# netease-youdao/EmotiVoice

Measured on AMD Instinct MI355X. Metric: mel_frames_per_sec, higher is better.
Workload: dtype f16+mxfp4 (fp32-class activations travelling as plane sets; per product one fp16 MFMA on the hi parts + two block-scaled MFMAs for the cross terms: fp4 x fp4 in every generator stage, the decoder's conv-FFN and QKV / output projections, fp4 weights x E5M2 activations in the fused 32-channel k = 3 pa

## Files before the change

emotivoice_amd/csrc/ev_gemm.hip:

```cpp
#include <hip/hip_fp16.h>
#include <stdlib.h>

#include "ev_kernels.h"
#include "ev_mxq.h"

#pragma clang fp contract(off)

namespace ev {

typedef _Float16 half8 __attribute__((ext_vector_type(8)));
typedef float f32x4 __attribute__((ext_vector_type(4)));
typedef float f32x2 __attribute__((ext_vector_type(2)));
typedef _Float16 half2v __attribute__((ext_vector_type(2)));

static constexpr int MAX_SPAN = 64;

__device__ __forceinline__ float max_raw(float a, float b) {
    float r;
    asm("v_max_f32 %0, %1, %2" : "=v"(r) : "v"(a), "v"(b));
    return r;
}
__device__ __forceinline__ float min_raw(float a, float b) {
    float r;
    asm("v_min_f32 %0, %1, %2" : "=v"(r) : "v"(a), "v"(b));
// ... 193 lines not shown
#define EV_TRACE_EPI_PARAMS
#define EV_TRACE_EPI_ARGS
#define EV_TRACE_EPI_DUMMY
#define EV_STAMP()
#endif

enum { EPI_RES16 = 1, EPI_RES32 = 2, EPI_ACC32 = 4, EPI_GENERIC = 8, EPI_RARE_ACT = 16, EPI_O16 = 32, EPI_O32 = 64, EPI_ADD16 = 128, EPI_LEAN = 256,
       EPI_MXP = 512, EPI_RESPL = 1024, EPI_ACCPL = 2048, EPI_PART = 4096 };

__device__ __forceinline__ float quad_xor1(float v) { return __builtin_bit_cast(float, __builtin_amdgcn_mov_dpp(__builtin_bit_cast(int, v), 0xB1, 0xF, 0xF, true)); }
__device__ __forceinline__ float quad_xor2(float v) { return __builtin_bit_cast(float, __builtin_amdgcn_mov_dpp(__builtin_bit_cast(int, v), 0x4E, 0xF, 0xF, true)); }
__device__ __forceinline__ void mx_quant8(const f32x2 (&a)[4], uint4& ho, unsigned& ch, unsigned& cl, unsigned& bh, unsigned& bl) {
    half2v hh[4];
    f32x2 hf[4], lf[4];
    float mh = 0.f, ml = 0.f;
#pragma unroll
    for (int j = 0; j < 4; ++j) {
        hh[j] = __builtin_convertvector(a[j], half2v);
        hf[j] = __builtin_convertvector(hh[j], f32x2);
        lf[j] = a[j] - hf[j];
        mh = max3_abs_raw(hf[j][0], hf[j][1], mh);
        ml = max3_abs_raw(lf[j][0], lf[j][1], ml);
    }
    mh = max_raw(mh, quad_xor1(mh)); mh = max_raw(mh, quad_xor2(mh));
    ml = max_raw(ml, quad_xor1(ml)); ml = max_raw(ml, quad_xor2(ml));
    bh = mx_scale_byte(mh); bl = mx_scale_byte(ml);
    const float sh = __uint_as_float(bh << 23), sl = __uint_as_float(bl << 23);
    ch = 0; cl = 0;
    ch = __builtin_amdgcn_cvt_scalef32_pk_fp4_f32(ch, hf[0][0], hf[0][1], sh, 0); cl = __builtin_amdgcn_cvt_scalef32_pk_fp4_f32(cl, lf[0][0], lf[0][1], sl, 0);
    ch = __builtin_amdgcn_cvt_scalef32_pk_fp4_f32(ch, hf[1][0], hf[1][1], sh, 1); cl = __builtin_amdgcn_cvt_scalef32_pk_fp4_f32(cl, lf[1][0], lf[1][1], sl, 1);
    ch = __builtin_amdgcn_cvt_scalef32_pk_fp4_f32(ch, hf[2][0], hf[2][1], sh, 2); cl = __builtin_amdgcn_cvt_scalef32_pk_fp4_f32(cl, lf[2][0], lf[2][1], sl, 2);
    ch = __builtin_amdgcn_cvt_scalef32_pk_fp4_f32(ch, hf[3][0], hf[3][1], sh, 3); cl = __builtin_amdgcn_cvt_scalef32_pk_fp4_f32(cl, lf[3][0], lf[3][1], sl, 3);
    ho.x = *reinterpret_cast<unsigned*>(&hh[0]); ho.y = *reinterpret_cast<unsigned*>(&hh[1]);
    ho.z = *reinterpret_cast<unsigned*>(&hh[2]); ho.w = *reinterpret_cast<unsigned*>(&hh[3]);
}
__device__ __forceinline__ long mx_scale_offset(const ConvGemmParams& p, long lin, long row_, int co) {
    const long row = p.mxo_logC ? (lin >> p.mxo_logC) : row_;
    const unsigned c = p.mxo_logC ? ((unsigned)lin & ((1u << p.mxo_logC) - 1u)) : (unsigned)co;
    return (long)(c >> 7) * p.mxo_qs_stride + row * 4 + ((c >> 5) & 3);
}
template <typename T>
__device__ __forceinline__ T* uptr(T* q) {
    unsigned long long b = reinterpret_cast<unsigned long long>(q);
    asm("" : "+s"(b));
    typedef __attribute__((address_space(1))) T* gptr;
    return (T*)(gptr)b;
}
__device__ __forceinline__ unsigned vlane(unsigned x) { asm volatile("" : "+v"(x)); return x; }
template <bool PART = false>
__device__ __forceinline__ void mx_emit_planes(const ConvGemmParams& p, const f32x2 (&a)[4], long ulin, unsigned llin_, long uso, unsigned lso_, int lane) {
    uint4 ho;
    unsigned ch, cl, bh, bl;
    mx_quant8(a, ho, ch, cl, bh, bl);
    const unsigned lh = vlane(llin_ * 2u), lq = vlane(llin_ >> 1), lso = vlane(lso_);
    char* const ph = uptr(reinterpret_cast<char*>(p.mxo_h) + ulin * 2);
    char* const pq0 = uptr(reinterpret_cast<char*>(p.mxo_q4[0]) + (ulin >> 1));
    char* const pq1 = uptr(reinterpret_cast<char*>(p.mxo_q4[1]) + (ulin >> 1));
#ifdef EV_MX_ABL
    const int abl = p.reserved0 >> 4;
    if (abl & 4) { if (p.M < 0) *reinterpret_cast<uint4*>(ph + lh) = uint4{ho.x ^ ch, ho.y ^ cl, ho.z ^ bh, ho.w ^ bl}; return; }
    if (abl & 8) { if (p.M < 0) ho.x ^= ch ^ cl ^ bh ^ bl; *reinterpret_cast<uint4*>(ph + lh) = ho; return; }
    if (abl & 16) {
        if (p.M < 0) ho.x ^= bh ^ bl;
        *reinterpret_cast<uint4*>(ph + lh) = ho;
        *reinterpret_cast<unsigned*>(pq0 + lq) = ch;
        *reinterpret_cast<unsigned*>(pq1 + lq) = cl;
        return;
    }
#endif
    *reinterpret_cast<uint4*>(ph + lh) = ho;
    if constexpr (!PART) *reinterpret_cast<unsigned*>(pq0 + lq) = ch;
    *reinterpret_cast<unsigned*>(pq1 + lq) = cl;
    if ((lane & 3) == 0) {
        if constexpr (!PART) uptr(reinterpret_cast<uint8_t*>(p.mxo_qs[0]) + uso)[lso] = (uint8_t)bh;
        uptr(reinterpret_cast<uint8_t*>(p.mxo_qs[1]) + uso)[lso] = (uint8_t)bl;
    }
}
__device__ __forceinline__ long uniform64(long v) {
    const unsigned lo = (unsigned)__builtin_amdgcn_readfirstlane((int)(unsigned)v), hi = (unsigned)__builtin_amdgcn_readfirstlane((int)(unsigned)((unsigned long)v >> 32));
    return (long)(((unsigned long)hi << 32) | lo);
}
__device__ uint8_t g_row_always_valid[4] = {1, 1, 1, 1};

template <int MT, int NT, int EPI, int RP = 32>
__device__ __forceinline__ void gemm_epilogue_fast(const ConvGemmParams& p, f32x4 (&acc)[NT][MT], char* wave_lds, int t0, int co0 EV_TRACE_EPI_PARAMS) {
    constexpr int TC = NT * 16;
    constexpr bool SWZ = RP == 16;
    constexpr int PITCH = SWZ ? TC * 4 : epi_pitch<TC>();
#ifdef EV_MXT
    unsigned long long mxt_e[12];
    int mxt_i = 0;
#define EV_MXT_STAMP() { __builtin_amdgcn_sched_barrier(0); mxt_e[mxt_i++] = __builtin_readcyclecounter(); __builtin_amdgcn_sched_barrier(0); }
#else
#define EV_MXT_STAMP()
#endif
    EV_MXT_STAMP()
    constexpr int LPR = TC / 8, RPI = 64 / LPR, IT = RP / RPI, NP = MT * 16 / RP, NG = MT / 2;
    static_assert((RP == 32 || (RP == 16 && TC == 64)) && IT >= 1, "rows per pass");
    int lane_ = threadIdx.x & 63;
    if constexpr (SWZ) asm volatile("" : "+v"(lane_));
    const int lane = lane_;
    const int fr = lane & 15, fq = lane >> 4;
    const int rr = lane / LPR, g = lane % LPR;
    const int co = co0 + g * 8;
    const int trow = t0 + rr;
    const int t0u = __builtin_amdgcn_readfirstlane(t0), co0u = __builtin_amdgcn_readfirstlane(co0);
    const unsigned l_o0 = (unsigned)(rr * p.ldo + g * 8), l_res0 = (unsigned)(rr * p.ldres + g * 8), l_acc0 = (unsigned)(rr * p.ldacc + g * 8),
                   l_add0 = (unsigned)(rr * p.ldadd + g * 8);
    const unsigned b_o32 = l_o0 * 4u, b_o16 = l_o0 * 2u, b_res16 = l_res0 * 2u, b_res32 = l_res0 * 4u, b_resq = l_res0 >> 1, b_acc = l_acc0 * 4u, b_add = l_add0 * 2u;
    const unsigned b_acc16 = l_acc0 * 2u, b_accq = l_acc0 >> 1;

    const uint8_t* vptr = p.row_valid ? p.row_valid : g_row_always_valid;
    const int vshift = p.row_valid ? p.valid_shift : 31;
    uint8_t vld[NG];
#pragma unroll
    for (int pass = 0; pass < NG; ++pass) vld[pass] = vptr[(t0 + pass * 32 + (lane & 31)) >> vshift];
    uint4 r16[2][IT], a16[2][IT][2];
    float4 r32[2][IT][2], a32[2][IT][2];
    uint4 rph[2][IT];
    unsigned rpc[2][IT], rps[2][IT];
    long rp_su = 0;
    unsigned rp_sl0 = 0;
    if constexpr (EPI & EPI_RESPL) {
        const long so = (long)(co >> 7) * p.res_xs_stride + ((co >> 5) & 3) + (long)rr * 4;
        rp_su = uniform64(so) + (long)t0u * 4;
        rp_sl0 = (unsigned)(so - uniform64(so));
    }
    uint4 aph[2][IT];
    unsigned apc[2][IT], aps[2][IT];
    long ap_su = 0;
    unsigned ap_sl0 = 0;
    if constexpr (EPI & EPI_ACCPL) {
        const long so = (long)(co >> 7) * p.acc_xs_stride + ((co >> 5) & 3) + (long)rr * 4;
        ap_su = uniform64(so) + (long)t0u * 4;
        ap_sl0 = (unsigned)(so - uniform64(so));
    }
    constexpr bool LEAN = (EPI & EPI_LEAN) != 0;
#define EV_EPI_RD(IT_, H) (SWZ ? ((IT_) * RPI + rr) * PITCH + (((2 * g + (H)) ^ (((IT_) * RPI + rr) & 15)) << 4) : ((IT_) * RPI + rr) * PITCH + g * 32 + (H) * 16)
#define EV_EPI_SET(PASS) (LEAN ? 0 : ((PASS) & 1))
#define EV_EPI_PREFETCH(PASS)                                                                                              \
    _Pragma("unroll") for (int it = 0; it < IT; ++it) {                                                                    \
        const long tu_ = t0u + (PASS) * RP + it * RPI;                                                                     \
        if constexpr (EPI & EPI_RES16)                                                                                     \
            r16[EV_EPI_SET(PASS)][it] = *reinterpret_cast<const uint4*>(uptr(reinterpret_cast<const char*>(p.res) + (tu_ * p.ldres + co0u) * 2) + vlane(b_res16)); \
        if constexpr (EPI & EPI_RES32) {                                                                                   \
            const char* rp_ = uptr(reinterpret_cast<const char*>(p.res) + (tu_ * p.ldres + co0u) * 4) + vlane(b_res32);    \
            r32[EV_EPI_SET(PASS)][it][0] = *reinterpret_cast<const float4*>(rp_);                                          \
            r32[EV_EPI_SET(PASS)][it][1] = *reinterpret_cast<const float4*>(rp_ + 16);                                     \
        }                                                                                                                  \
        if constexpr (EPI & EPI_RESPL) {                                                                                   \
            const long ulin_ = tu_ * p.ldres + co0u;                                                                       \
            rph[EV_EPI_SET(PASS)][it] = *reinterpret_cast<const uint4*>(uptr(reinterpret_cast<const char*>(p.res) + ulin_ * 2) + vlane(b_res16));  \
            rpc[EV_EPI_SET(PASS)][it] = *reinterpret_cast<const unsigned*>(uptr(reinterpret_cast<const char*>(p.res_x4) + (ulin_ >> 1)) + vlane(b_resq)); \
            rps[EV_EPI_SET(PASS)][it] = uptr(reinterpret_cast<const uint8_t*>(p.res_xs) + (rp_su + ((PASS) * RP + it * RPI) * 4))[vlane(rp_sl0)]; \
        }                                                                                                                  \
        if constexpr (EPI & EPI_ACCPL) {                                                                                   \
            const long ulin_ = tu_ * p.ldacc + co0u;                                                                       \
            aph[EV_EPI_SET(PASS)][it] = *reinterpret_cast<const uint4*>(uptr(reinterpret_cast<const char*>(p.acc_h) + ulin_ * 2) + vlane(b_acc16));  \
            apc[EV_EPI_SET(PASS)][it] = *reinterpret_cast<const unsigned*>(uptr(reinterpret_cast<const char*>(p.acc_x4) + (ulin_ >> 1)) + vlane(b_accq)); \
            aps[EV_EPI_SET(PASS)][it] = uptr(reinterpret_cast<const uint8_t*>(p.acc_xs) + (ap_su + ((PASS) * RP + it * RPI) * 4))[vlane(ap_sl0)]; \
        }                                                                                                                  \
        if constexpr (EPI & EPI_ACC32) {                                                                                   \
            const char* ap_ = uptr(reinterpret_cast<const char*>(p.acc32) + (tu_ * p.ldacc + co0u) * 4) + vlane(b_acc);    \
            a32[EV_EPI_SET(PASS)][it][0] = *reinterpret_cast<const float4*>(ap_);                                          \
            a32[EV_EPI_SET(PASS)][it][1] = *reinterpret_cast<const float4*>(ap_ + 16);                                     \
        }                                                                                                                  \
        if constexpr (EPI & EPI_ADD16) {                                                                                   \
            a16[EV_EPI_SET(PASS)][it][0] = *reinterpret_cast<const uint4*>(uptr(reinterpret_cast<const char*>(p.add16_a) + (tu_ * p.ldadd + co0u) * 2) + vlane(b_add)); \
            a16[EV_EPI_SET(PASS)][it][1] = *reinterpret_cast<const uint4*>(uptr(reinterpret_cast<const char*>(p.add16_b) + (tu_ * p.ldadd + co0u) * 2) + vlane(b_add)); \
        }                                                                                                                  \
    }
    if constexpr (!LEAN) { EV_EPI_PREFETCH(0) }
    unsigned vmask[NG];
#pragma unroll
    for (int pass = 0; pass < NG; ++pass) vmask[pass] = (unsigned)__builtin_amdgcn_ballot_w64(vld[pass] != 0);

    f32x2 bias2[4];
#pragma unroll
    for (int j = 0; j < 4; ++j) bias2[j] = f32x2{0.f, 0.f};
    if (p.bias) {
        const float4 b0 = *reinterpret_cast<const float4*>(p.bias + co), b1 = *reinterpret_cast<const float4*>(p.bias + co + 4);
        bias2[0] = f32x2{b0.x, b0.y}; bias2[1] = f32x2{b0.z, b0.w}; bias2[2] = f32x2{b1.x, b1.y}; bias2[3] = f32x2{b1.z, b1.w};
    }
    const int act = p.act;
    const f32x2 act_slope2 = f32x2{p.act_slope, p.act_slope};
    const f32x2 out_scale2 = f32x2{p.out_scale, p.out_scale};
    const bool has_post = p.post_lrelu != 0;
    const f32x2 post_slope2 = f32x2{p.post_slope, p.post_slope};
    const f32x2 mxo_slope2 = f32x2{p.mxo_slope, p.mxo_slope};
    const f32x2 res_inv2 = f32x2{p.res_inv_slope, p.res_inv_slope};
    const bool mxo_act = __float_as_uint(p.mxo_slope) != 0x3f800000u, scaled = __float_as_uint(p.out_scale) != 0x3f800000u;
    __half* const o16 = reinterpret_cast<__half*>(p.out16);
    float* const o32a = p.out32_before_post ? p.out32 : nullptr;
    float* const o32b = p.out32_before_post ? nullptr : p.out32;
    const long rowoff_u = (long)t0u * p.ldo + co0u;
    unsigned lrbit[32 / RPI];
#pragma unroll
    for (int it = 0; it < 32 / RPI; ++it) lrbit[it] = 1u << (it * RPI + rr);
    long mx_su = 0;
    unsigned mx_sl = 0;
    int mx_sstep = 0;
    if constexpr (EPI & EPI_MXP) {
        static_assert(TC == 64, "plane-set epilogue: 64-channel wave tiles");
        const long so = mx_scale_offset(p, rowoff_u + l_o0, (long)trow, co);
        mx_su = uniform64(so);
        mx_sl = (unsigned)(so - mx_su);
        mx_sstep = 4 * (p.mxo_logC ? (p.ldo >> p.mxo_logC) : 1);
    }
    EV_STAMP()
    EV_MXT_STAMP()

#pragma unroll
    for (int pass = 0; pass < NP; ++pass) {
#ifdef EV_MXT
        if constexpr (SWZ) {
            if (p.reserved0 & 4) {
                const bool late = (threadIdx.x >> 8) != 0;
                if (pass == 0) { if (late) __builtin_amdgcn_s_setprio(1); }
                if (pass == NP / 2) { if (late) __builtin_amdgcn_s_setprio(0); else __builtin_amdgcn_s_setprio(1); }
            }
        }
#endif
        __builtin_amdgcn_wave_barrier();
        if constexpr (LEAN) { EV_EPI_PREFETCH(pass) }
        if constexpr (SWZ) {
#pragma unroll
            for (int a = 0; a < NT; ++a)
                *reinterpret_cast<f32x4*>(wave_lds + fr * PITCH + (((a * 4 + fq) ^ fr) << 4)) = acc[a][pass];
        } else {
#pragma unroll
            for (int bb = 0; bb < 2; ++bb)
#pragma unroll
                for (int a = 0; a < NT; ++a)
                    *reinterpret_cast<f32x4*>(wave_lds + (bb * 16 + fr) * PITCH + (a * 16 + 4 * fq) * 4) = acc[a][pass * 2 + bb];
        }
        __builtin_amdgcn_wave_barrier();
        if constexpr (!LEAN) { if (pass + 1 < NP) { EV_EPI_PREFETCH(pass + 1) } }
        EV_STAMP()
        f32x4 lv[IT][2];
        if constexpr (!LEAN) {
#pragma unroll
            for (int it = 0; it < IT; ++it) {
                lv[it][0] = *reinterpret_cast<const f32x4*>(wave_lds + EV_EPI_RD(it, 0));
                lv[it][1] = *reinterpret_cast<const f32x4*>(wave_lds + EV_EPI_RD(it, 1));
            }
        }
#pragma unroll
        for (int it = 0; it < IT; ++it) {
            if constexpr (LEAN) {
                lv[it][0] = *reinterpret_cast<const f32x4*>(wave_lds + EV_EPI_RD(it, 0));
                lv[it][1] = *reinterpret_cast<const f32x4*>(wave_lds + EV_EPI_RD(it, 1));
            }
            const long off_u = rowoff_u + (long)(pass * RP + it * RPI) * p.ldo;
            const f32x4 v0 = lv[it][0], v1 = lv[it][1];
            f32x2 v[4] = {f32x2{v0[0], v0[1]}, f32x2{v0[2], v0[3]}, f32x2{v1[0], v1[1]}, f32x2{v1[2], v1[3]}};
#pragma unroll
            for (int j = 0; j < 4; ++j) v[j] += bias2[j];
            if constexpr (EPI & EPI_RARE_ACT) {
                if (act == ACT_GELU && (EPI & (EPI_O16 | EPI_MXP)) && !(EPI & EPI_O32)) {
#pragma unroll
                    for (int j = 0; j < 4; ++j) { v[j][0] = gelu_fast(v[j][0]); v[j][1] = gelu_fast(v[j][1]); }
                } else {
#pragma unroll
                    for (int j = 0; j < 4; ++j) { v[j][0] = apply_act(v[j][0], act, 0.f); v[j][1] = apply_act(v[j][1], act, 0.f); }
                }
            } else if (act == ACT_LRELU) {
#pragma unroll
                for (int j = 0; j < 4; ++j) v[j] = lrelu2(v[j], act_slope2);
            }
            if constexpr (EPI & EPI_RES16) {
                const half2v* h = reinterpret_cast<const half2v*>(&r16[EV_EPI_SET(pass)][it]);
#pragma unroll
                for (int j = 0; j < 4; ++j) v[j] += __builtin_convertvector(h[j], f32x2);
            }
            if constexpr (EPI & EPI_RES32) {
                const float4 r0 = r32[EV_EPI_SET(pass)][it][0], r1 = r32[EV_EPI_SET(pass)][it][1];
                v[0] += f32x2{r0.x, r0.y}; v[1] += f32x2{r0.z, r0.w}; v[2] += f32x2{r1.x, r1.y}; v[3] += f32x2{r1.z, r1.w};
            }
            if constexpr (EPI & EPI_RESPL) {
                const half2v* h = reinterpret_cast<const half2v*>(&rph[EV_EPI_SET(pass)][it]);
                const unsigned cw = rpc[EV_EPI_SET(pass)][it];
                const float sc = __uint_as_float(rps[EV_EPI_SET(pass)][it] << 23);
                f32x2 a[4];
                a[0] = __builtin_convertvector(h[0], f32x2) + __builtin_amdgcn_cvt_scalef32_pk_f32_fp4(cw, sc, 0);
                a[1] = __builtin_convertvector(h[1], f32x2) + __builtin_amdgcn_cvt_scalef32_pk_f32_fp4(cw, sc, 1);
                a[2] = __builtin_convertvector(h[2], f32x2) + __builtin_amdgcn_cvt_scalef32_pk_f32_fp4(cw, sc, 2);
                a[3] = __builtin_convertvector(h[3], f32x2) + __builtin_amdgcn_cvt_scalef32_pk_f32_fp4(cw, sc, 3);
#pragma unroll
                for (int j = 0; j < 4; ++j) {
                    const f32x2 t = a[j] * res_inv2;
                    v[j] += f32x2{min_raw(a[j][0], t[0]), min_raw(a[j][1], t[1])};
                }
            }
            if (scaled) {
                asm volatile("" ::: "memory");
#pragma unroll
                for (int j = 0; j < 4; ++j) v[j] *= out_scale2;
            }
            if constexpr (EPI & EPI_ACC32) {
                const float4 r0 = a32[EV_EPI_SET(pass)][it][0], r1 = a32[EV_EPI_SET(pass)][it][1];
                v[0] += f32x2{r0.x, r0.y}; v[1] += f32x2{r0.z, r0.w}; v[2] += f32x2{r1.x, r1.y}; v[3] += f32x2{r1.z, r1.w};
            }
            if constexpr (EPI & EPI_ACCPL) {
                const half2v* h = reinterpret_cast<const half2v*>(&aph[EV_EPI_SET(pass)][it]);
                const unsigned cw = apc[EV_EPI_SET(pass)][it];
// ... 1858 lines not shown
```

emotivoice_amd/csrc/ev_gemm_mx64.h:

```cpp
#pragma once

template <int TAPS>
struct Mx64Sched {
    static constexpr int KG = (TAPS + 1) / 2, KH = (KG + 1) / 2, KP = KG * 2, NS = 2 * KG + 2 * KH;
    static constexpr int chunk_of(int s) { return s < KG ? 0 : (s < 2 * KG ? 1 : (s < 2 * KG + KH ? 2 : 3)); }
    static constexpr int first_of(int c) { return c == 0 ? 0 : (c == 1 ? KG : (c == 2 ? 2 * KG : 2 * KG + KH)); }
    static constexpr bool starts_chunk(int s) { return s == first_of(chunk_of(s)); }
    static constexpr int x_issued(int t) { return (starts_chunk(t) && chunk_of(t) < 3) ? 3 : 0; }
    static constexpr int w_issued(int t) { return t + 3 < NS ? 1 : 0; }
    static constexpr int issued_before(int t) {
        int n = 6;
        for (int j = 0; j < t; ++j) n += x_issued(j) + w_issued(j);
        return n;
    }
    static constexpr int idx_w(int m) { return m < 3 ? 3 + m : issued_before(m - 3) + x_issued(m - 3); }
    static constexpr int idx_xlast(int c) { return c == 0 ? 2 : issued_before(first_of(c - 1)) + 2; }
    static constexpr int wait_imm(int s) {
        if (s + 1 >= NS) return -1;
        int need = idx_w(s + 1);
        if (starts_chunk(s + 1)) { const int x = idx_xlast(chunk_of(s + 1)); need = x > need ? x : need; }
        return issued_before(s) - 1 - need;
    }
};
static_assert(Mx64Sched<11>::NS == 18 && Mx64Sched<7>::NS == 12 && Mx64Sched<11>::wait_imm(0) == 1 && Mx64Sched<11>::wait_imm(1) == 4 && Mx64Sched<11>::wait_imm(2) == 1, "schedule");

template <int N> __device__ __forceinline__ void mx64_wait() {
    if constexpr (N >= 0) asm volatile("s_waitcnt vmcnt(%0)" ::"n"(N) : "memory");
}

template <int TAPS, int EPI>
__global__ __launch_bounds__(512, 4) void conv_gemm_mx64_kernel(const ConvGemmParams p) {
    using SC = Mx64Sched<TAPS>;
    constexpr int BM = PH_BM, XBUF = PH_XBUF, WBUF = PH_WBUF, MT = 2, NT = 4, KG = SC::KG, KP = SC::KP, NS = SC::NS;
    static_assert(PH_SLABR >= BM + MAX_SPAN + 64 && KP * 128 <= 2048 && (TAPS == 7 || TAPS == 11), "slab rows / weight-scale run / tap counts");
    extern __shared__ __attribute__((aligned(16))) char smem[];
    char* const Xs = smem;
    char* const Ws = smem + 2 * XBUF;
    const int tid = threadIdx.x, lane = tid & 63;
    const int wave = __builtin_amdgcn_readfirstlane(tid >> 6);
    const int wc = wave >> 2;
    const unsigned lds0 = (unsigned)(size_t)(__attribute__((address_space(3))) char*)smem;

    int bid = blockIdx.x;
    {
        const int nblk = gridDim.x, q = nblk >> 3, r = nblk & 7, xcd = bid & 7, local = bid >> 3;
        bid = (xcd < r ? xcd * (q + 1) : r * (q + 1) + (xcd - r) * q) + local;
    }
    const int m0 = bid * BM;
    const int dil = p.dil;
    const int row0 = m0 - p.center * dil;
    const int row0a = row0 & ~3, soff = row0 - row0a;
    const int last_row = BM + (TAPS - 1) * dil - 1;

    const int prow = lane >> 2;
    const unsigned pp16 = (unsigned)(((lane & 3) ^ ((lane >> 3) & 3)) << 4);
    const int wco = (wave & 3) * 16 + prow;
    const unsigned w16_lane = (unsigned)wco * (unsigned)(TAPS * 128) + pp16;
    const unsigned wq = (unsigned)((lane & 3) ^ ((lane >> 3) & 3));
    const unsigned w4_lane = (unsigned)(((wco >> 5) * KP + (int)(wq >> 1)) * 1024 + (wco & 31) * 32 + (int)(wq & 1) * 16);
    unsigned x16_lane[3], x4_lane[2];
#pragma unroll
    for (int i = 0; i < 3; ++i) x16_lane[i] = (unsigned)min((wave + 8 * i) * 16 + prow, last_row) * 128u + pp16;
#pragma unroll
    for (int i = 0; i < 2; ++i) x4_lane[i] = (unsigned)min((wave + 8 * i) * 32 + (lane >> 1), last_row) * 32u + (unsigned)(lane & 1) * 16u;
    const int xs_run = ((BM + (TAPS - 1) * dil + soff) * 4 + 15) & ~15;
    unsigned sc_lane;
    if (wave == 4) sc_lane = min(lane * 16, xs_run - 16);
    else if (wave == 5) sc_lane = min(1024 + lane * 16, xs_run - 16);
    else if (wave == 6) sc_lane = min(lane * 16, KP * 128 - 16);
    else sc_lane = min(1024 + lane * 16, KP * 128 - 16);

    const char* const wmx = reinterpret_cast<const char*>(p.W_mx);
    constexpr int WQB = KP * 32 * 32 * 2, WSB = KP * 32 * 2 * 2;
    const char* const xb16 = uniform_ptr(reinterpret_cast<const char*>(p.A) + (long)row0 * 128L);
    const char* const xb4[2] = {uniform_ptr(reinterpret_cast<const char*>(p.mx_x4[0]) + (long)row0 * 32L), uniform_ptr(reinterpret_cast<const char*>(p.mx_x4[1]) + (long)row0 * 32L)};
    const char* const xsb[2] = {uniform_ptr(reinterpret_cast<const char*>(p.mx_xs[0]) + (long)row0a * 4L), uniform_ptr(reinterpret_cast<const char*>(p.mx_xs[1]) + (long)row0a * 4L)};
    const char* const wb16 = uniform_ptr(reinterpret_cast<const char*>(p.W));
    const unsigned xdst = __builtin_amdgcn_readfirstlane(lds0 + wave * 1024), wdst = xdst + 2 * XBUF;

    auto issue_x = [&](auto cc) {
        constexpr int C_ = decltype(cc)::value;
        constexpr unsigned dst = (unsigned)((C_ & 1) * XBUF);
        if constexpr (C_ < 2) {
#pragma unroll
            for (int i = 0; i < 3; ++i) glds16(xb16 + C_ * 64, x16_lane[i], xdst + dst + i * 8192);
        } else {
            constexpr int P_ = C_ - 2;
            glds16(xb4[P_], x4_lane[0], xdst + dst);
            glds16(xb4[P_], x4_lane[1], xdst + dst + 8192);
            const bool sc = wave >= 4;
            const char* const sbase = wave < 6 ? xsb[P_] : wmx + 2 * WQB + P_ * WSB;
            glds16(sc ? sbase : xb4[P_], sc ? sc_lane : x4_lane[1], xdst + dst + 2 * 8192);
        }
    };
    auto issue_w = [&](auto ss) {
        constexpr int S_ = decltype(ss)::value;
        constexpr int C_ = SC::chunk_of(S_), U_ = S_ - SC::first_of(C_);
        const int sel = wave >> 2;
        if constexpr (C_ < 2) {
            const int t = min(2 * U_ + sel, TAPS - 1);
            glds16(wb16 + C_ * 64 + (unsigned)t * 128u, w16_lane, wdst + (S_ & 3) * WBUF);
        } else {
            const int g = min(2 * U_ + sel, KG - 1);
            glds16(wmx + (C_ - 2) * WQB + (unsigned)(2 * g) * 1024u, w4_lane, wdst + (S_ & 3) * WBUF);
        }
    };

    f32x4 acc[NT][MT];
#pragma unroll
    for (int a = 0; a < NT; ++a)
#pragma unroll
        for (int b = 0; b < MT; ++b) acc[a][b] = f32x4{0.f, 0.f, 0.f, 0.f};
    const int fr = lane & 15, fq = lane >> 4;

    bool tile_live = true;
    if (p.row_valid) {
        const uint8_t* vp = p.row_valid;
        const int r4 = m0 + lane * 4, vs = p.valid_shift;
        const unsigned any = vp[r4 >> vs] | vp[(r4 + 1) >> vs] | vp[(r4 + 2) >> vs] | vp[(r4 + 3) >> vs];
        tile_live = __builtin_amdgcn_ballot_w64(any != 0) != 0ull;
    }
    if (tile_live) {
        issue_x(std::integral_constant<int, 0>{});
        issue_w(std::integral_constant<int, 0>{});
        issue_w(std::integral_constant<int, 1>{});
        issue_w(std::integral_constant<int, 2>{});
        asm volatile("s_waitcnt vmcnt(0)" ::: "memory");
        __builtin_amdgcn_s_barrier();
        if (wc == 1) __builtin_amdgcn_s_barrier();

        const int xrow = wave * 32 + fr;
        const int x4row = xrow + (fq >> 1) * dil;
        const int xs_base = MX_XS_OFF + soff * 4 + (fq & 1);
        int ws_lane[NT];
#pragma unroll
        for (int a = 0; a < NT; ++a) {
            const int co = a * 16 + fr;
            ws_lane[a] = MX_WS_OFF + (((co >> 5) * KP + (fq >> 1)) * 32 + (co & 31)) * 2 + (fq & 1);
        }

#define EV_MX64_STEP(S)                                                                                                              \
    if constexpr ((S) < NS) {                                                                                                        \
        constexpr int C_ = SC::chunk_of(S), U_ = (S) - SC::first_of(C_);                                                             \
        const char* const Xb = Xs + (C_ & 1) * XBUF;                                                                                 \
        const char* const Wb = Ws + ((S) & 3) * WBUF;                                                                                \
        uint4 xf[2][MT], wf[2][NT];                                                                                                  \
        int xsc[2][MT], wsc[2][NT];                                                                                                  \
        constexpr int NSEL = (C_ < 2) ? ((2 * U_ + 1 < TAPS) ? 2 : 1) : ((2 * U_ + 1 < KG) ? 2 : 1);                                 \
        int dil_ = dil;                                                                                                              \
        asm volatile("" : "+s"(dil_));                                                                                               \
        _Pragma("unroll") for (int sel = 0; sel < NSEL; ++sel) {                                                                     \
            _Pragma("unroll") for (int a = 0; a < NT; ++a) wf[sel][a] = *reinterpret_cast<const uint4*>(Wb + swz(sel * 64 + a * 16 + fr, fq)); \
            if constexpr (C_ < 2) {                                                                                                  \
                const int r_ = xrow + (2 * U_ + sel) * dil_;                                                                         \
                _Pragma("unroll") for (int b = 0; b < MT; ++b) {                                                                     \
                    const int rb_ = r_ + b * 16;                                                                                     \
                    xf[sel][b] = *reinterpret_cast<const uint4*>(Xb + rb_ * 64 + ((fq ^ ((rb_ >> 1) & 3)) << 4));                    \
                }                                                                                                                    \
            } else {                                                                                                                 \
                const int g_ = 2 * U_ + sel;                                                                                         \
                const int r_ = x4row + 2 * g_ * dil_;                                                                                \
                _Pragma("unroll") for (int b = 0; b < MT; ++b) {                                                                     \
                    xf[sel][b] = *reinterpret_cast<const uint4*>(Xb + (r_ + b * 16) * 32 + ((fq & 1) << 4));                         \
                    xsc[sel][b] = *reinterpret_cast<const uint8_t*>(Xb + xs_base + (r_ + b * 16) * 4);                               \
                }                                                                                                                    \
                _Pragma("unroll") for (int a = 0; a < NT; ++a) wsc[sel][a] = *reinterpret_cast<const uint8_t*>(Xb + ws_lane[a] + g_ * 128); \
            }                                                                                                                        \
        }                                                                                                                            \
        mx64_wait<SC::wait_imm(S)>();                                                                                                \
        __builtin_amdgcn_sched_barrier(0);                                                                                           \
        __builtin_amdgcn_s_barrier();                                                                                                \
        __builtin_amdgcn_sched_barrier(0);                                                                                           \
        __builtin_amdgcn_s_setprio(1);                                                                                               \
        _Pragma("unroll") for (int sel = 0; sel < NSEL; ++sel)                                                                       \
            _Pragma("unroll") for (int a = 0; a < NT; ++a)                                                                           \
                _Pragma("unroll") for (int b = 0; b < MT; ++b) {                                                                     \
                    if constexpr (C_ < 2) mfma_inplace(acc[a][b], *reinterpret_cast<half8*>(&wf[sel][a]), *reinterpret_cast<half8*>(&xf[sel][b])); \
                    else mfma_mx_inplace(acc[a][b], wf[sel][a], xf[sel][b], wsc[sel][a], xsc[sel][b]);                               \
                    const int idx = (sel * NT + a) * MT + b;                                                                         \
                    if constexpr (SC::x_issued(S) != 0) { if (idx == 2) issue_x(std::integral_constant<int, (C_ < 3 ? C_ + 1 : 3)>{}); } \
                    if constexpr (SC::w_issued(S) != 0) { if (idx == 5) issue_w(std::integral_constant<int, ((S) + 3 < NS ? (S) + 3 : 0)>{}); } \
                }                                                                                                                    \
        __builtin_amdgcn_s_setprio(0);                                                                                               \
        __builtin_amdgcn_sched_barrier(0);                                                                                           \
        __builtin_amdgcn_s_barrier();                                                                                                \
        __builtin_amdgcn_sched_barrier(0);                                                                                           \
    }
        EV_MX64_STEP(0) EV_MX64_STEP(1) EV_MX64_STEP(2) EV_MX64_STEP(3) EV_MX64_STEP(4) EV_MX64_STEP(5)
        EV_MX64_STEP(6) EV_MX64_STEP(7) EV_MX64_STEP(8) EV_MX64_STEP(9) EV_MX64_STEP(10) EV_MX64_STEP(11)
        EV_MX64_STEP(12) EV_MX64_STEP(13) EV_MX64_STEP(14) EV_MX64_STEP(15) EV_MX64_STEP(16) EV_MX64_STEP(17)
#undef EV_MX64_STEP
        asm volatile("s_waitcnt vmcnt(0)" ::: "memory");
        if (wc == 0) __builtin_amdgcn_s_barrier();
        __builtin_amdgcn_s_barrier();
        mfma_asm_fence(acc);
    }
    if constexpr (EPI == EPI_GENERIC) gemm_epilogue_lds<MT, NT>(p, acc, smem + wave * epi_wave_bytes<64>(), m0 + wave * 32, 0);
    else {
        EV_TRACE_EPI_DUMMY
        gemm_epilogue_fast<MT, NT, EPI, 16>(p, acc, smem + wave * 4096, m0 + wave * 32, 0 EV_TRACE_EPI_ARGS);
    }
}

template <int TAPS, int EPI>
static void launch_mx64_epi(const ConvGemmParams& p, hipStream_t s) {
    hipLaunchKernelGGL((conv_gemm_mx64_kernel<TAPS, EPI>), dim3(p.M / PH_BM), dim3(512), PH_LDS, s, p);
}
template <int TAPS>
static void launch_mx64_taps(const ConvGemmParams& p, int e, hipStream_t s) {
    switch (e) {
#define EV_MX64_CASE(E) case (E): launch_mx64_epi<TAPS, (E)>(p, s); break;
        EV_MX_VARIANTS(EV_MX64_CASE)
#undef EV_MX64_CASE
        default: break;
    }
}
template <int TAPS>
static hipError_t mx64_attr_taps() {
    hipError_t e = hipSuccess, r;
#define EV_MX64_ATTR(E) r = hipFuncSetAttribute((const void*)conv_gemm_mx64_kernel<TAPS, (E)>, hipFuncAttributeMaxDynamicSharedMemorySize, (int)PH_LDS); if (r != hipSuccess) e = r;
    EV_MX_VARIANTS(EV_MX64_ATTR)
#undef EV_MX64_ATTR
    return e;
}
static hipError_t mx64_set_attributes() {
    hipError_t e = hipSuccess, r;
    r = mx64_attr_taps<7>(); if (r != hipSuccess) e = r;
    r = mx64_attr_taps<11>(); if (r != hipSuccess) e = r;
    return e;
}
static bool mx64_eligible(const ConvGemmParams& p) {
    return p.W_mx && p.N == 64 && p.K == 64 && p.lda == 64 && (p.taps == 11 || p.taps == 7) && p.M % PH_BM == 0 && (p.taps - 1) * p.dil <= MAX_SPAN &&
           p.center * 2 == p.taps - 1 && p.mx_x4[0] && p.mx_x4[1] && p.mx_xs[0] && p.mx_xs[1] && !p.pro_lrelu && !(p.reserved0 & 8) && mx_epi_variant(p) >= 0;
}
static void launch_mx64(const ConvGemmParams& p, hipStream_t s) {
    if (p.taps == 7) launch_mx64_taps<7>(p, mx_epi_variant(p), s); else launch_mx64_taps<11>(p, mx_epi_variant(p), s);
}
```

Before: 726,900.

## Add 384-row tile variant of mx64 conv GEMM with reworked load schedule

```diff
diff --git a/emotivoice_amd/csrc/ev_gemm.hip b/emotivoice_amd/csrc/ev_gemm.hip
--- a/emotivoice_amd/csrc/ev_gemm.hip
+++ b/emotivoice_amd/csrc/ev_gemm.hip
@@ -299,7 +299,7 @@
 }
 __device__ uint8_t g_row_always_valid[4] = {1, 1, 1, 1};
 
-template <int MT, int NT, int EPI, int RP = 32>
+template <int MT, int NT, int EPI, int RP = 32, bool MLIM = false>
 __device__ __forceinline__ void gemm_epilogue_fast(const ConvGemmParams& p, f32x4 (&acc)[NT][MT], char* wave_lds, int t0, int co0 EV_TRACE_EPI_PARAMS) {
     constexpr int TC = NT * 16;
     constexpr bool SWZ = RP == 16;
@@ -312,8 +312,8 @@
 #define EV_MXT_STAMP()
 #endif
     EV_MXT_STAMP()
-    constexpr int LPR = TC / 8, RPI = 64 / LPR, IT = RP / RPI, NP = MT * 16 / RP, NG = MT / 2;
-    static_assert((RP == 32 || (RP == 16 && TC == 64)) && IT >= 1, "rows per pass");
+    constexpr int LPR = TC / 8, RPI = 64 / LPR, IT = RP / RPI, NP = MT * 16 / RP, NG = (MT + 1) / 2;
+    static_assert((RP == 32 || (RP == 16 && TC == 64)) && IT >= 1 && (MT % 2 == 0 || RP == 16) && (!MLIM || RP == 16), "rows per pass");
     int lane_ = threadIdx.x & 63;
     if constexpr (SWZ) asm volatile("" : "+v"(lane_));
     const int lane = lane_;
@@ -331,7 +331,7 @@
     const int vshift = p.row_valid ? p.valid_shift : 31;
     uint8_t vld[NG];
 #pragma unroll
-    for (int pass = 0; pass < NG; ++pass) vld[pass] = vptr[(t0 + pass * 32 + (lane & 31)) >> vshift];
+    for (int pass = 0; pass < NG; ++pass) vld[pass] = vptr[(MLIM ? min(t0 + pass * 32 + (lane & 31), p.M - 1) : t0 + pass * 32 + (lane & 31)) >> vshift];
     uint4 r16[2][IT], a16[2][IT][2];
     float4 r32[2][IT][2], a32[2][IT][2];
     uint4 rph[2][IT];
@@ -357,7 +357,8 @@
 #define EV_EPI_SET(PASS) (LEAN ? 0 : ((PASS) & 1))
 #define EV_EPI_PREFETCH(PASS)                                                                                              \
     _Pragma("unroll") for (int it = 0; it < IT; ++it) {                                                                    \
-        const long tu_ = t0u + (PASS) * RP + it * RPI;                                                                     \
+        const int du_ = MLIM ? min(t0u + (PASS) * RP + it * RPI, p.M - RPI) - t0u : (PASS) * RP + it * RPI;                \
+        const long tu_ = t0u + du_;                                                                                        \
         if constexpr (EPI & EPI_RES16)                                                                                     \
             r16[EV_EPI_SET(PASS)][it] = *reinterpret_cast<const uint4*>(uptr(reinterpret_cast<const char*>(p.res) + (tu_ * p.ldres + co0u) * 2) + vlane(b_res16)); \
         if constexpr (EPI & EPI_RES32) {                                                                                   \
@@ -369,13 +370,13 @@
             const long ulin_ = tu_ * p.ldres + co0u;                                                                       \
             rph[EV_EPI_SET(PASS)][it] = *reinterpret_cast<const uint4*>(uptr(reinterpret_cast<const char*>(p.res) + ulin_ * 2) + vlane(b_res16));  \
             rpc[EV_EPI_SET(PASS)][it] = *reinterpret_cast<const unsigned*>(uptr(reinterpret_cast<const char*>(p.res_x4) + (ulin_ >> 1)) + vlane(b_resq)); \
-            rps[EV_EPI_SET(PASS)][it] = uptr(reinterpret_cast<const uint8_t*>(p.res_xs) + (rp_su + ((PASS) * RP + it * RPI) * 4))[vlane(rp_sl0)]; \
+            rps[EV_EPI_SET(PASS)][it] = uptr(reinterpret_cast<const uint8_t*>(p.res_xs) + (rp_su + du_ * 4))[vlane(rp_sl0)]; \
         }                                                                                                                  \
         if constexpr (EPI & EPI_ACCPL) {                                                                                   \
             const long ulin_ = tu_ * p.ldacc + co0u;                                                                       \
             aph[EV_EPI_SET(PASS)][it] = *reinterpret_cast<const uint4*>(uptr(reinterpret_cast<const char*>(p.acc_h) + ulin_ * 2) + vlane(b_acc16));  \
             apc[EV_EPI_SET(PASS)][it] = *reinterpret_cast<const unsigned*>(uptr(reinterpret_cast<const char*>(p.acc_x4) + (ulin_ >> 1)) + vlane(b_accq)); \
-            aps[EV_EPI_SET(PASS)][it] = uptr(reinterpret_cast<const uint8_t*>(p.acc_xs) + (ap_su + ((PASS) * RP + it * RPI) * 4))[vlane(ap_sl0)]; \
+            aps[EV_EPI_SET(PASS)][it] = uptr(reinterpret_cast<const uint8_t*>(p.acc_xs) + (ap_su + du_ * 4))[vlane(ap_sl0)]; \
         }                                                                                                                  \
         if constexpr (EPI & EPI_ACC32) {                                                                                   \
             const char* ap_ = uptr(reinterpret_cast<const char*>(p.acc32) + (tu_ * p.ldacc + co0u) * 4) + vlane(b_acc);    \
@@ -438,6 +439,7 @@
             }
         }
 #endif
+        if constexpr (MLIM) { if (t0u + pass * RP >= p.M) break; }
         __builtin_amdgcn_wave_barrier();
         if constexpr (LEAN) { EV_EPI_PREFETCH(pass) }
         if constexpr (SWZ) {
diff --git a/emotivoice_amd/csrc/ev_gemm_mx64.h b/emotivoice_amd/csrc/ev_gemm_mx64.h
--- a/emotivoice_amd/csrc/ev_gemm_mx64.h
+++ b/emotivoice_amd/csrc/ev_gemm_mx64.h
@@ -1,20 +1,23 @@
 #pragma once
 
-template <int TAPS>
+template <int TAPS, int MT_ = 2>
 struct Mx64Sched {
     static constexpr int KG = (TAPS + 1) / 2, KH = (KG + 1) / 2, KP = KG * 2, NS = 2 * KG + 2 * KH;
+    static constexpr int XP16 = MT_ == 3 ? 4 : 3, XP4 = 3, WD = MT_ == 3 ? 2 : 3;
+    static constexpr bool W_FIRST = MT_ == 3;
+    static constexpr int pieces(int c) { return c < 2 ? XP16 : XP4; }
     static constexpr int chunk_of(int s) { return s < KG ? 0 : (s < 2 * KG ? 1 : (s < 2 * KG + KH ? 2 : 3)); }
     static constexpr int first_of(int c) { return c == 0 ? 0 : (c == 1 ? KG : (c == 2 ? 2 * KG : 2 * KG + KH)); }
     static constexpr bool starts_chunk(int s) { return s == first_of(chunk_of(s)); }
-    static constexpr int x_issued(int t) { return (starts_chunk(t) && chunk_of(t) < 3) ? 3 : 0; }
-    static constexpr int w_issued(int t) { return t + 3 < NS ? 1 : 0; }
+    static constexpr int x_issued(int t) { return (starts_chunk(t) && chunk_of(t) < 3) ? pieces(chunk_of(t) + 1) : 0; }
+    static constexpr int w_issued(int t) { return t + WD < NS ? 1 : 0; }
     static constexpr int issued_before(int t) {
-        int n = 6;
+        int n = pieces(0) + WD;
         for (int j = 0; j < t; ++j) n += x_issued(j) + w_issued(j);
         return n;
     }
-    static constexpr int idx_w(int m) { return m < 3 ? 3 + m : issued_before(m - 3) + x_issued(m - 3); }
-    static constexpr int idx_xlast(int c) { return c == 0 ? 2 : issued_before(first_of(c - 1)) + 2; }
+    static constexpr int idx_w(int m) { return m < WD ? pieces(0) + m : issued_before(m - WD) + (W_FIRST ? 0 : x_issued(m - WD)); }
+    static constexpr int idx_xlast(int c) { return c == 0 ? pieces(0) - 1 : issued_before(first_of(c - 1)) + (W_FIRST ? w_issued(first_of(c - 1)) : 0) + pieces(c) - 1; }
     static constexpr int wait_imm(int s) {
         if (s + 1 >= NS) return -1;
         int need = idx_w(s + 1);
@@ -23,16 +26,22 @@
     }
 };
 static_assert(Mx64Sched<11>::NS == 18 && Mx64Sched<7>::NS == 12 && Mx64Sched<11>::wait_imm(0) == 1 && Mx64Sched<11>::wait_imm(1) == 4 && Mx64Sched<11>::wait_imm(2) == 1, "schedule");
+static_assert(Mx64Sched<11, 3>::wait_imm(0) == 0 && Mx64Sched<11, 3>::wait_imm(1) == 4 && Mx64Sched<11, 3>::wait_imm(2) == 0 && Mx64Sched<11, 3>::wait_imm(5) == 0 &&
+              Mx64Sched<7, 3>::wait_imm(1) == 4 && Mx64Sched<7, 3>::wait_imm(3) == 0, "schedule, 384 rows");
+
+static constexpr int MX64_XBUF384 = (384 + MAX_SPAN) * 64;
 
 template <int N> __device__ __forceinline__ void mx64_wait() {
     if constexpr (N >= 0) asm volatile("s_waitcnt vmcnt(%0)" ::"n"(N) : "memory");
 }
 
-template <int TAPS, int EPI>
+template <int TAPS, int EPI, int MT = 2>
 __global__ __launch_bounds__(512, 4) void conv_gemm_mx64_kernel(const ConvGemmParams p) {
-    using SC = Mx64Sched<TAPS>;
-    constexpr int BM = PH_BM, XBUF = PH_XBUF, WBUF = PH_WBUF, MT = 2, NT = 4, KG = SC::KG, KP = SC::KP, NS = SC::NS;
-    static_assert(PH_SLABR >= BM + MAX_SPAN + 64 && KP * 128 <= 2048 && (TAPS == 7 || TAPS == 11), "slab rows / weight-scale run / tap counts");
+    using SC = Mx64Sched<TAPS, MT>;
+    constexpr bool R384 = MT == 3;
+    constexpr int BM = MT * 128, XBUF = R384 ? MX64_XBUF384 : PH_XBUF, WBUF = PH_WBUF, NT = 4, KG = SC::KG, KP = SC::KP, NS = SC::NS, NSLOT = SC::WD + 1;
+    static_assert((MT == 2 || MT == 3) && XBUF >= (BM + MAX_SPAN) * 64 && (BM + MAX_SPAN) * 32 <= 16384 && (BM + MAX_SPAN + 3) * 4 <= 2048 && MX_XS_OFF + 4096 <= XBUF &&
+                  2 * XBUF + NSLOT * WBUF <= (int)PH_LDS && KP * 128 <= 2048 && (TAPS == 7 || TAPS == 11), "slab rows / scale runs / LDS / tap counts");
     extern __shared__ __attribute__((aligned(16))) char smem[];
     char* const Xs = smem;
     char* const Ws = smem + 2 * XBUF;
@@ -50,7 +59,8 @@
     const int dil = p.dil;
     const int row0 = m0 - p.center * dil;
     const int row0a = row0 & ~3, soff = row0 - row0a;
-    const int last_row = BM + (TAPS - 1) * dil - 1;
+    const int tile_rows = R384 ? min(BM, p.M - m0) : BM;
+    const int last_row = tile_rows + (TAPS - 1) * dil - 1;
 
     const int prow = lane >> 2;
     const unsigned pp16 = (unsigned)(((lane & 3) ^ ((lane >> 3) & 3)) << 4);
@@ -58,12 +68,14 @@
     const unsigned w16_lane = (unsigned)wco * (unsigned)(TAPS * 128) + pp16;
     const unsigned wq = (unsigned)((lane & 3) ^ ((lane >> 3) & 3));
     const unsigned w4_lane = (unsigned)(((wco >> 5) * KP + (int)(wq >> 1)) * 1024 + (wco & 31) * 32 + (int)(wq & 1) * 16);
-    unsigned x16_lane[3], x4_lane[2];
-#pragma unroll
-    for (int i = 0; i < 3; ++i) x16_lane[i] = (unsigned)min((wave + 8 * i) * 16 + prow, last_row) * 128u + pp16;
+    constexpr int XP16 = SC::XP16;
+    const int x16_p3 = wave >= 4 ? 2 : 3;
+    unsigned x16_lane[XP16], x4_lane[2];
+#pragma unroll
+    for (int i = 0; i < XP16; ++i) x16_lane[i] = (unsigned)min((wave + 8 * (i == 3 ? x16_p3 : i)) * 16 + prow, last_row) * 128u + pp16;
 #pragma unroll
     for (int i = 0; i < 2; ++i) x4_lane[i] = (unsigned)min((wave + 8 * i) * 32 + (lane >> 1), last_row) * 32u + (unsigned)(lane & 1) * 16u;
-    const int xs_run = ((BM + (TAPS - 1) * dil + soff) * 4 + 15) & ~15;
+    const int xs_run = ((tile_rows + (TAPS - 1) * dil + soff) * 4 + 15) & ~15;
     unsigned sc_lane;
     if (wave == 4) sc_lane = min(lane * 16, xs_run - 16);
     else if (wave == 5) sc_lane = min(1024 + lane * 16, xs_run - 16);
@@ -83,7 +95,7 @@
         constexpr unsigned dst = (unsigned)((C_ & 1) * XBUF);
         if constexpr (C_ < 2) {
 #pragma unroll
-            for (int i = 0; i < 3; ++i) glds16(xb16 + C_ * 64, x16_lane[i], xdst + dst + i * 8192);
+            for (int i = 0; i < XP16; ++i) glds16(xb16 + C_ * 64, x16_lane[i], xdst + dst + (i == 3 ? x16_p3 : i) * 8192);
         } else {
             constexpr int P_ = C_ - 2;
             glds16(xb4[P_], x4_lane[0], xdst + dst);
@@ -99,10 +111,10 @@
         const int sel = wave >> 2;
         if constexpr (C_ < 2) {
             const int t = min(2 * U_ + sel, TAPS - 1);
-            glds16(wb16 + C_ * 64 + (unsigned)t * 128u, w16_lane, wdst + (S_ & 3) * WBUF);
+            glds16(wb16 + C_ * 64 + (unsigned)t * 128u, w16_lane, wdst + (S_ % NSLOT) * WBUF);
         } else {
             const int g = min(2 * U_ + sel, KG - 1);
-            glds16(wmx + (C_ - 2) * WQB + (unsigned)(2 * g) * 1024u, w4_lane, wdst + (S_ & 3) * WBUF);
+            glds16(wmx + (C_ - 2) * WQB + (unsigned)(2 * g) * 1024u, w4_lane, wdst + (S_ % NSLOT) * WBUF);
         }
     };
 
@@ -111,25 +123,40 @@
     for (int a = 0; a < NT; ++a)
 #pragma unroll
         for (int b = 0; b < MT; ++b) acc[a][b] = f32x4{0.f, 0.f, 0.f, 0.f};
+    if constexpr (R384) {
+#pragma unroll
+        for (int a = 0; a < NT; ++a)
+#pragma unroll
+            for (int b = 0; b < MT; ++b) asm volatile("" : "+v"(acc[a][b]));
+    }
     const int fr = lane & 15, fq = lane >> 4;
 
     bool tile_live = true;
     if (p.row_valid) {
         const uint8_t* vp = p.row_valid;
-        const int r4 = m0 + lane * 4, vs = p.valid_shift;
-        const unsigned any = vp[r4 >> vs] | vp[(r4 + 1) >> vs] | vp[(r4 + 2) >> vs] | vp[(r4 + 3) >> vs];
+        const int vs = p.valid_shift;
+        unsigned any;
+        if constexpr (R384) {
+            const int r6 = m0 + lane * 6, rl = p.M - 1;
+            any = 0;
+#pragma unroll
+            for (int i = 0; i < 6; ++i) any |= vp[min(r6 + i, rl) >> vs];
+        } else {
+            const int r4 = m0 + lane * 4;
+            any = vp[r4 >> vs] | vp[(r4 + 1) >> vs] | vp[(r4 + 2) >> vs] | vp[(r4 + 3) >> vs];
+        }
         tile_live = __builtin_amdgcn_ballot_w64(any != 0) != 0ull;
     }
     if (tile_live) {
         issue_x(std::integral_constant<int, 0>{});
         issue_w(std::integral_constant<int, 0>{});
         issue_w(std::integral_constant<int, 1>{});
-        issue_w(std::integral_constant<int, 2>{});
+        if constexpr (SC::WD > 2) issue_w(std::integral_constant<int, 2>{});
         asm volatile("s_waitcnt vmcnt(0)" ::: "memory");
         __builtin_amdgcn_s_barrier();
         if (wc == 1) __builtin_amdgcn_s_barrier();
 
-        const int xrow = wave * 32 + fr;
+        const int xrow = wave * (MT * 16) + fr;
         const int x4row = xrow + (fq >> 1) * dil;
         const int xs_base = MX_XS_OFF + soff * 4 + (fq & 1);
         int ws_lane[NT];
@@ -143,7 +170,7 @@
     if constexpr ((S) < NS) {                                                                                                        \
         constexpr int C_ = SC::chunk_of(S), U_ = (S) - SC::first_of(C_);                                                             \
         const char* const Xb = Xs + (C_ & 1) * XBUF;                                                                                 \
-        const char* const Wb = Ws + ((S) & 3) * WBUF;                                                                                \
+        const char* const Wb = Ws + ((S) % NSLOT) * WBUF;                                                                            \
         uint4 xf[2][MT], wf[2][NT];                                                                                                  \
         int xsc[2][MT], wsc[2][NT];                                                                                                  \
         constexpr int NSEL = (C_ < 2) ? ((2 * U_ + 1 < TAPS) ? 2 : 1) : ((2 * U_ + 1 < KG) ? 2 : 1);                                 \
@@ -186,19 +213,87 @@
         __builtin_amdgcn_s_barrier();                                                                                                \
         __builtin_amdgcn_sched_barrier(0);                                                                                           \
     }
+#define EV_MX64_LDW(SEL, A_)                                                                                                         \
+        { wf[A_] = *reinterpret_cast<const uint4*>(Wb + swz((SEL) * 64 + (A_) * 16 + fr, fq));                                       \
+          if constexpr (C_ >= 2) wsc[A_] = *reinterpret_cast<const uint8_t*>(Xb + ws_lane[A_] + (2 * U_ + (SEL)) * 128); }
+#define EV_MX64_LDX(DST, DSC, SEL, B_)                                                                                               \
+        { if constexpr (C_ < 2) {                                                                                                    \
+              const int rb_ = xrow + (2 * U_ + (SEL)) * dil_ + (B_) * 16;                                                            \
+              DST = *reinterpret_cast<const uint4*>(Xb + rb_ * 64 + ((fq ^ ((rb_ >> 1) & 3)) << 4));                                 \
+          } else {                                                                                                                   \
+              const int rb_ = x4row + 2 * (2 * U_ + (SEL)) * dil_ + (B_) * 16;                                                       \
+              DST = *reinterpret_cast<const uint4*>(Xb + rb_ * 32 + ((fq & 1) << 4));                                                \
+              DSC = *reinterpret_cast<const uint8_t*>(Xb + xs_base + rb_ * 4);                                                       \
+          } }
+#define EV_MX64_MMA(A_, XF, XS)                                                                                                      \
+        { if constexpr (C_ < 2) mfma_inplace(acc[A_][b], *reinterpret_cast<half8*>(&wf[A_]), *reinterpret_cast<half8*>(&XF));         \
+          else mfma_mx_inplace(acc[A_][b], wf[A_], XF, wsc[A_], XS); }
+#define EV_MX64_STEP3(S)                                                                                                             \
+    if constexpr ((S) < NS) {                                                                                                        \
+        constexpr int C_ = SC::chunk_of(S), U_ = (S) - SC::first_of(C_);                                                             \
+        const char* const Xb = Xs + (C_ & 1) * XBUF;                                                                                 \
+        const char* const Wb = Ws + ((S) % NSLOT) * WBUF;                                                                            \
+        uint4 xf[MT], xg[MT], wf[NT];                                                                                                \
+        int xsc[MT], xgc[MT], wsc[NT];                                                                                               \
+        constexpr int NSEL = (C_ < 2) ? ((2 * U_ + 1 < TAPS) ? 2 : 1) : ((2 * U_ + 1 < KG) ? 2 : 1);                                 \
+        int dil_ = dil;                                                                                                              \
+        asm volatile("" : "+s"(dil_));                                                                                               \
+        _Pragma("unroll") for (int a = 0; a < NT; ++a) EV_MX64_LDW(0, a)                                                             \
+        _Pragma("unroll") for (int b = 0; b < MT; ++b) EV_MX64_LDX(xf[b], xsc[b], 0, b)                                              \
+        mx64_wait<SC::wait_imm(S)>();                                                                                                \
+        __builtin_amdgcn_sched_barrier(0);                                                                                           \
+        __builtin_amdgcn_s_barrier();                                                                                                \
+        __builtin_amdgcn_sched_barrier(0);                                                                                           \
+        __builtin_amdgcn_s_setprio(1);                                                                                               \
+        _Pragma("unroll") for (int a = 0; a < NT; ++a) {                                                                             \
+            _Pragma("unroll") for (int b = 0; b < MT; ++b) {                                                                         \
+                EV_MX64_MMA(a, xf[b], xsc[b])                                                                                        \
+                const int idx = a * MT + b;                                                                                          \
+                if constexpr (SC::w_issued(S) != 0) { if (idx == 1) issue_w(std::integral_constant<int, ((S) + SC::WD < NS ? (S) + SC::WD : 0)>{}); } \
+                if constexpr (SC::x_issued(S) != 0) { if (idx == 4) issue_x(std::integral_constant<int, (C_ < 3 ? C_ + 1 : 3)>{}); } \
+            }                                                                                                                        \
+            if constexpr (NSEL == 2) {                                                                                               \
+                __builtin_amdgcn_sched_barrier(0);                                                                                   \
+                EV_MX64_LDW(1, a)                                                                                                    \
+                if (a == NT - 2) EV_MX64_LDX(xg[0], xgc[0], 1, 0)                                                                    \
+                if (a == NT - 1) { _Pragma("unroll") for (int b = 1; b < MT; ++b) EV_MX64_LDX(xg[b], xgc[b], 1, b) }                 \
+                __builtin_amdgcn_sched_barrier(0);                                                                                   \
+            }                                                                                                                        \
+        }                                                                                                                            \
+        if constexpr (NSEL == 2) {                                                                                                   \
+            _Pragma("unroll") for (int b = 0; b < MT; ++b)                                                                           \
+                _Pragma("unroll") for (int a = 0; a < NT; ++a) EV_MX64_MMA(a, xg[b], xgc[b])                                         \
+        }                                                                                                                            \
+        __builtin_amdgcn_s_setprio(0);                                                                                               \
+        __builtin_amdgcn_sched_barrier(0);                                                                                           \
+        __builtin_amdgcn_s_barrier();                                                                                                \
+        __builtin_amdgcn_sched_barrier(0);                                                                                           \
+    }
+        if constexpr (!R384) {
         EV_MX64_STEP(0) EV_MX64_STEP(1) EV_MX64_STEP(2) EV_MX64_STEP(3) EV_MX64_STEP(4) EV_MX64_STEP(5)
         EV_MX64_STEP(6) EV_MX64_STEP(7) EV_MX64_STEP(8) EV_MX64_STEP(9) EV_MX64_STEP(10) EV_MX64_STEP(11)
         EV_MX64_STEP(12) EV_MX64_STEP(13) EV_MX64_STEP(14) EV_MX64_STEP(15) EV_MX64_STEP(16) EV_MX64_STEP(17)
+        } else {
+        EV_MX64_STEP3(0) EV_MX64_STEP3(1) EV_MX64_STEP3(2) EV_MX64_STEP3(3) EV_MX64_STEP3(4) EV_MX64_STEP3(5)
+        EV_MX64_STEP3(6) EV_MX64_STEP3(7) EV_MX64_STEP3(8) EV_MX64_STEP3(9) EV_MX64_STEP3(10) EV_MX64_STEP3(11)
+        EV_MX64_STEP3(12) EV_MX64_STEP3(13) EV_MX64_STEP3(14) EV_MX64_STEP3(15) EV_MX64_STEP3(16) EV_MX64_STEP3(17)
+        }
 #undef EV_MX64_STEP
+#undef EV_MX64_STEP3
+#undef EV_MX64_MMA
+#undef EV_MX64_LDX
+#undef EV_MX64_LDW
         asm volatile("s_waitcnt vmcnt(0)" ::: "memory");
         if (wc == 0) __builtin_amdgcn_s_barrier();
         __builtin_amdgcn_s_barrier();
         mfma_asm_fence(acc);
     }
-    if constexpr (EPI == EPI_GENERIC) gemm_epilogue_lds<MT, NT>(p, acc, smem + wave * epi_wave_bytes<64>(), m0 + wave * 32, 0);
-    else {
+    if constexpr (EPI == EPI_GENERIC) {
+        static_assert(EPI != EPI_GENERIC || !R384, "the generic epilogue stores whole tiles");
+        gemm_epilogue_lds<MT, NT>(p, acc, smem + wave * epi_wave_bytes<64>(), m0 + wave * 32, 0);
+    } else {
         EV_TRACE_EPI_DUMMY
-        gemm_epilogue_fast<MT, NT, EPI, 16>(p, acc, smem + wave * 4096, m0 + wave * 32, 0 EV_TRACE_EPI_ARGS);
+        gemm_epilogue_fast<MT, NT, EPI, 16, R384>(p, acc, smem + wave * 4096, m0 + wave * (MT * 16), 0 EV_TRACE_EPI_ARGS);
     }
 }
 
@@ -206,8 +301,29 @@
 static void launch_mx64_epi(const ConvGemmParams& p, hipStream_t s) {
     hipLaunchKernelGGL((conv_gemm_mx64_kernel<TAPS, EPI>), dim3(p.M / PH_BM), dim3(512), PH_LDS, s, p);
 }
+#define EV_MX64_VARIANTS_384(X) X(EPI_MXP) X(EPI_RESPL | EPI_LEAN | EPI_MXP) X(EPI_RESPL | EPI_LEAN | EPI_MXP | EPI_PART) \
+    X(EPI_RESPL | EPI_ACCPL | EPI_LEAN | EPI_MXP | EPI_PART) X(EPI_RESPL | EPI_ACCPL | EPI_LEAN | EPI_MXP)
+static bool mx64_form_384(int e) {
+    switch (e) {
+#define EV_MX64_IS384(E) case (E): return true;
+        EV_MX64_VARIANTS_384(EV_MX64_IS384)
+#undef EV_MX64_IS384
+        default: return false;
+    }
+}
+template <int TAPS>
+static void launch_mx64_taps_384(const ConvGemmParams& p, int e, hipStream_t s) {
+    const int grid = (p.M + 383) / 384;
+    switch (e) {
+#define EV_MX64_CASE384(E) case (E): hipLaunchKernelGGL((conv_gemm_mx64_kernel<TAPS, (E), 3>), dim3(grid), dim3(512), PH_LDS, s, p); break;
+        EV_MX64_VARIANTS_384(EV_MX64_CASE384)
+#undef EV_MX64_CASE384
+        default: break;
+    }
+}
 template <int TAPS>
 static void launch_mx64_taps(const ConvGemmParams& p, int e, hipStream_t s) {
+    if (mx64_form_384(e) && !(p.reserved0 & 2048)) { launch_mx64_taps_384<TAPS>(p, e, s); return; }
     switch (e) {
 #define EV_MX64_CASE(E) case (E): launch_mx64_epi<TAPS, (E)>(p, s); break;
         EV_MX_VARIANTS(EV_MX64_CASE)
@@ -221,6 +337,9 @@
 #define EV_MX64_ATTR(E) r = hipFuncSetAttribute((const void*)conv_gemm_mx64_kernel<TAPS, (E)>, hipFuncAttributeMaxDynamicSharedMemorySize, (int)PH_LDS); if (r != hipSuccess) e = r;
     EV_MX_VARIANTS(EV_MX64_ATTR)
 #undef EV_MX64_ATTR
+#define EV_MX64_ATTR384(E) r = hipFuncSetAttribute((const void*)conv_gemm_mx64_kernel<TAPS, (E), 3>, hipFuncAttributeMaxDynamicSharedMemorySize, (int)PH_LDS); if (r != hipSuccess) e = r;
+    EV_MX64_VARIANTS_384(EV_MX64_ATTR384)
+#undef EV_MX64_ATTR384
     return e;
 }
 static hipError_t mx64_set_attributes() {
```

Result: no change. 733,100, median of 6 (+0.9%).
